# SteveMacenski/slam_toolbox

Measured on NVIDIA B200. Metric: scan matches/sec (1081-beam, +-2m/+-20deg), higher is better.
Workload: dtype u8

## Files before the change

### slam_toolbox_b200/csrc/sm_tile.cu

```cuda
#include <algorithm>
#include <cmath>
#include <cstdlib>
#include <cstring>
#include <type_traits>
#include <vector>

#include "common.cuh"
#include "sm_math.cuh"
#include "sm_types.cuh"
#include "sm_device.cuh"
#include "sm_sweep_dev.cuh"

namespace b200 {

constexpr int kRowTiles = 6;
constexpr int kYTile = 8 * kRowTiles;
constexpr int kChunkBeams = 640;

__device__ __forceinline__ uint32_t smem_u32(const void * p) { return (uint32_t)__cvta_generic_to_shared(p); }
__device__ __forceinline__ void mbar_init(uint32_t bar, uint32_t count)
{
  asm volatile("mbarrier.init.shared::cta.b64 [%0], %1;" ::"r"(bar), "r"(count) : "memory");
}
__device__ __forceinline__ void mbar_expect_tx(uint32_t bar, uint32_t bytes)
{
  asm volatile("mbarrier.arrive.expect_tx.shared::cta.b64 _, [%0], %1;" ::"r"(bar), "r"(bytes) : "memory");
}
__device__ __forceinline__ void bulk_g2s(uint32_t dst, const void * src, uint32_t bytes, uint32_t bar)
{
  asm volatile("cp.async.bulk.shared::cluster.global.mbarrier::complete_tx::bytes [%0], [%1], %2, [%3];" ::"r"(dst), "l"(src),
               "r"(bytes), "r"(bar)
               : "memory");
}
__device__ __forceinline__ void mbar_wait(uint32_t bar, uint32_t parity)
{
  uint32_t done = 0;
  while (!done) {
    asm volatile(
      "{\n\t.reg .pred p;\n\tmbarrier.try_wait.parity.shared::cta.b64 p, [%1], %2;\n\tselp.u32 %0, 1, 0, p;\n\t}"
      : "=r"(done)
      : "r"(bar), "r"(parity)
      : "memory");
  }
}
__device__ __forceinline__ uint32_t cluster_rank()
{
  uint32_t r;
  asm volatile("mov.u32 %0, %%cluster_ctarank;" : "=r"(r));
  return r;
}
__device__ __forceinline__ void cluster_arrive() { asm volatile("barrier.cluster.arrive.release.aligned;" ::: "memory"); }
__device__ __forceinline__ void cluster_wait() { asm volatile("barrier.cluster.wait.acquire.aligned;" ::: "memory"); }
__device__ __forceinline__ uint32_t dsmem_addr(const void * local, uint32_t rank)
{
  uint32_t r;
  asm volatile("mapa.shared::cluster.u32 %0, %1, %2;" : "=r"(r) : "r"(smem_u32(local)), "r"(rank));
  return r;
}
__device__ __forceinline__ void dsmem_st_f64(uint32_t a, double v) { asm volatile("st.shared::cluster.f64 [%0], %1;" ::"r"(a), "d"(v) : "memory"); }
__device__ __forceinline__ void dsmem_st_s32(uint32_t a, int v) { asm volatile("st.shared::cluster.s32 [%0], %1;" ::"r"(a), "r"(v) : "memory"); }
__device__ __forceinline__ int dsmem_ld_s32(uint32_t a)
{
  int v;
  asm volatile("ld.shared::cluster.s32 %0, [%1];" : "=r"(v) : "r"(a) : "memory");
  return v;
}
__device__ __forceinline__ double dsmem_ld_f64(uint32_t a)
{
  double v;
  asm volatile("ld.shared::cluster.f64 %0, [%1];" : "=d"(v) : "r"(a) : "memory");
  return v;
}

__device__ __forceinline__ uint32_t lds_u32(uint32_t a)
{
  uint32_t v;
  asm volatile("ld.shared.u32 %0, [%1];" : "=r"(v) : "r"(a));
  return v;
}

__device__ __forceinline__ uint32_t even_bytes_t(uint32_t w) { return __byte_perm(w, 0, 0x4240); }
__device__ __forceinline__ uint32_t odd_bytes_t(uint32_t w) { return __byte_perm(w, 0, 0x4341); }

struct TieRes {
  double L;
  double L2;
  int cnt;
  int sum0;
  int ties[kMaxTies];
};

__device__ void tie_merge(TieRes & a, const double bL, const double bL2, const int bcnt, const int bsum0, const int * bties)
{
  if (bL == a.L) {
    int out[kMaxTies];
    const int na = a.cnt < kMaxTies ? a.cnt : kMaxTies, nb = bcnt < kMaxTies ? bcnt : kMaxTies;
    int i = 0, j = 0, k = 0;
    while (k < kMaxTies && (i < na || j < nb)) {
      if (j >= nb || (i < na && a.ties[i] < bties[j])) out[k++] = a.ties[i++];
      else out[k++] = bties[j++];
    }
    if (nb > 0 && (na == 0 || bties[0] < a.ties[0])) a.sum0 = bsum0;
    for (int t = 0; t < k; ++t) a.ties[t] = out[t];
    a.cnt += bcnt;
    a.L2 = bL2 > a.L2 ? bL2 : a.L2;
  } else if (bL > a.L) {
    double l2 = a.L > a.L2 ? a.L : a.L2;
    l2 = bL2 > l2 ? bL2 : l2;
    a.L = bL; a.L2 = l2; a.cnt = bcnt; a.sum0 = bsum0;
    const int nb = bcnt < kMaxTies ? bcnt : kMaxTies;
    for (int t = 0; t < nb; ++t) a.ties[t] = bties[t];
// ... 111 lines not shown
        for (int lv = 0; lv < (nlev > 0 ? nlev : 1); ++lv) {
          const uint32_t want = nlev > 0 ? f.level[lv] : 0u;
          for (int it = it0; it < it1; ++it) {
            const int32_t * cl = it == it0 ? cells0 : d.cells + (size_t)it * d.max_n;
            const int ncell = it == it0 ? ncell0 : d.cell_count[it];
            for (int t = tid; t < ncell; t += kTileThreads) {
              const int32_t cell = cl[t];
              if (cell < 0) continue;
              const int cx = (cell & 0xFFFF) + d.roi_x - half, cy = (cell >> 16) + d.roi_y - half;
              for (int ky = (cy ^ pq) & 1; ky < d.ksize; ky += 2) {
                const int rel = ((cy + ky) >> 1) - band_r0;
                if ((unsigned)rel >= (unsigned)f.alloc_rows) continue;
                for (int kx = (cx ^ pp) & 1; kx < d.ksize; kx += 2) {
                  const uint32_t kv = kern[ky * d.ksize + kx];
                  if (nlev > 0) { if (kv == want) S8[rel * pitchB + ((cx + kx) >> 1)] = (uint8_t)kv; }
                  else if (kv) atomic_max_u8(S8 + rel * pitchB + ((cx + kx) >> 1), kv);
                }
              }
            }
          }
          if (lv + 1 < nlev) __syncthreads();
        }
      }
      if (e.flags & (kSeqNewChunk | kSeqNewStage)) __syncthreads();
      if (tid == 0) {
        const TileSeq * nxt = nullptr;
        if (si + 1 < nseq) nxt = seq + si + 1;
        else if (pair + nclusters < d.npairs) nxt = f.seq + f.seq_start[d.pair_query[pair + nclusters] * C + rank];
        if (nxt) issue(nxt, (cnt + 1) & 1);
      }
      mbar_wait(bar0 + 8 * (cnt & 1), (cnt >> 1) & 1);
      const unsigned char * stg = s_raw + f.off_stage + (size_t)(cnt & 1) * f.stage_bytes;
      const int32_t * tbl = reinterpret_cast<const int32_t *>(stg);
      const uint8_t * order = stg + (size_t)e.na * 48;
      const uint16_t * pay = reinterpret_cast<const uint16_t *>(stg + (((size_t)e.na * 52 + 15) & ~(size_t)15));
      const int tiles = f.ytiles * f.xtiles;
      const int nitems = e.na * 4 * tiles;
      const bool has_edge = (e.flags & kSeqHasEdge) != 0;
      for (;;) {
        int item = 0;
        if (lane == 0) item = atomicAdd(&sh.ctr[cnt & 1], 1);
        item = __shfl_sync(0xffffffffu, item, 0);
        if (item >= nitems) break;
        const int gi = item / tiles, ti = item - gi * tiles;
        const int g = order[gi];
        const int al = g >> 2, m = g & 3;
        const int yt = ti / f.xtiles, xt = ti - yt * f.xtiles;
        const int a = e.a0 + al;
        int32_t * Arow = A + (size_t)(a - chunk_a0) * P;
        const int ybase = y_l + kYTile * yt;
       {
        int b = tbl[(al * 4 + m) * 3 + 0];
        const int mb = tbl[(al * 4 + m) * 3 + 1], me = tbl[(al * 4 + m) * 3 + 2];
        const int pe = mb;
        int eb = 0, ee = 0;
        if (has_edge) {
          const int32_t * es = f.edge_start + (((size_t)q * nA + a) * 4 * nb + e.stage) * 4 + m;
          eb = es[0]; ee = es[1];
        }
        if (b == pe && mb == me && eb == ee) break;
        uint32_t base = smem_u32(S8) + (uint32_t)(((y_l + kYTile * yt) * pitch_w + 4 * xt + j_l) * 4);
        asm volatile("" : "+r"(base));
        const int x0 = 4 * (4 * xt + j_l) - m;
        auto flush = [&](const uint32_t (&T0)[kRowTiles], const uint32_t (&T1)[kRowTiles]) {
          uint32_t any = 0;
#pragma unroll
          for (int r = 0; r < kRowTiles; ++r) any |= T0[r] | T1[r];
          if (!__any_sync(0xffffffffu, any != 0)) return;
#pragma unroll
          for (int r = 0; r < kRowTiles; ++r) {
            const int y = ybase + 8 * r;
            if (y >= nY || (T0[r] | T1[r]) == 0) continue;
            int32_t * dst = Arow + y * nX + x0;
            const int v0 = T0[r] & 0xFFFF, v1 = T1[r] & 0xFFFF, v2 = T0[r] >> 16, v3 = T1[r] >> 16;
            if (v0 && (unsigned)(x0 + 0) < (unsigned)nX) atomicAdd(dst + 0, v0);
            if (v1 && (unsigned)(x0 + 1) < (unsigned)nX) atomicAdd(dst + 1, v1);
            if (v2 && (unsigned)(x0 + 2) < (unsigned)nX) atomicAdd(dst + 2, v2);
            if (v3 && (unsigned)(x0 + 3) < (unsigned)nX) atomicAdd(dst + 3, v3);
          }
        };
        bool multi_done = (mb == me);
        if (b < pe || !multi_done) {
          do {
            const int ce = min(pe, b + kChunkBeams);
            uint32_t T0[kRowTiles], T1[kRowTiles];
#pragma unroll
            for (int r = 0; r < kRowTiles; ++r) { T0[r] = 0; T1[r] = 0; }
            for (; b + 3 < ce; b += 4) {
              const uint2 dd = *reinterpret_cast<const uint2 *>(pay + b);
              const uint32_t o0 = base + 4u * __byte_perm(dd.x, 0, 0x4410), o1 = base + 4u * __byte_perm(dd.x, 0, 0x4432);
              const uint32_t o2 = base + 4u * __byte_perm(dd.y, 0, 0x4410), o3 = base + 4u * __byte_perm(dd.y, 0, 0x4432);
#pragma unroll
              for (int r = 0; r < kRowTiles; ++r) {
                const uint32_t wa = lds_u32(o0 + r * 8 * pitchB) +
                                    lds_u32(o1 + r * 8 * pitchB);
                const uint32_t wb = lds_u32(o2 + r * 8 * pitchB) +
                                    lds_u32(o3 + r * 8 * pitchB);
                T0[r] = T0[r] + even_bytes_t(wa) + even_bytes_t(wb);
                T1[r] = T1[r] + odd_bytes_t(wa) + odd_bytes_t(wb);
              }
            }
            for (; b + 1 < ce; b += 2) {
              const uint32_t dd = *reinterpret_cast<const uint32_t *>(pay + b);
              const uint32_t o0 = base + ((dd & 0xFFFFu) << 2), o1 = base + ((dd >> 16) << 2);
#pragma unroll
              for (int r = 0; r < kRowTiles; ++r) {
                const uint32_t w = lds_u32(o0 + r * 8 * pitchB) +
                                   lds_u32(o1 + r * 8 * pitchB);
                T0[r] += even_bytes_t(w);
                T1[r] += odd_bytes_t(w);
              }
            }
            if (b < ce) {
              const uint32_t o0 = base + ((uint32_t)pay[b] << 2);
#pragma unroll
              for (int r = 0; r < kRowTiles; ++r) {
                const uint32_t w = lds_u32(o0 + r * 8 * pitchB);
                T0[r] += even_bytes_t(w);
                T1[r] += odd_bytes_t(w);
              }
              ++b;
            }
            if (b == pe && !multi_done) {
              for (int k = mb; k < me; k += 2) {
                const uint32_t dm = *reinterpret_cast<const uint32_t *>(pay + k);
                const uint32_t o0 = base + ((dm & 0xFFFFu) << 2);
                const uint32_t kk = dm >> 16;
#pragma unroll
                for (int r = 0; r < kRowTiles; ++r) {
                  const uint32_t w = lds_u32(o0 + r * 8 * pitchB);
                  T0[r] += even_bytes_t(w) * kk;
                  T1[r] += odd_bytes_t(w) * kk;
                }
              }
              multi_done = true;
            }
            flush(T0, T1);
          } while (b < pe || !multi_done);
        }
        while (eb < ee) {
          const int ce = min(ee, eb + kChunkBeams);
          uint32_t T0[kRowTiles], T1[kRowTiles];
#pragma unroll
          for (int r = 0; r < kRowTiles; ++r) { T0[r] = 0; T1[r] = 0; }
          for (int b0 = eb; b0 < ce; b0 += 32) {
            const int cn = min(32, ce - b0);
            const int32_t mine = (lane < cn) ? f.edge[b0 + lane] : 0;
            for (int k = 0; k < cn; ++k) {
              const int32_t ev = __shfl_sync(0xffffffffu, mine, k);
              const int row0 = (int)(int16_t)(ev & 0xFFFF) + ybase, wq = (ev >> 16) + 4 * xt + j_l;
              const bool cv = (unsigned)wq < (unsigned)pitch_w;
#pragma unroll
              for (int r = 0; r < kRowTiles; ++r) {
                const int row = row0 + 8 * r;
                const uint32_t w = (cv && (unsigned)row < (unsigned)f.alloc_rows) ? S[row * pitch_w + wq] : 0u;
                T0[r] += even_bytes_t(w);
                T1[r] += odd_bytes_t(w);
              }
            }
          }
          eb = ce;
          flush(T0, T1);
        }
       }
      }
      if (e.flags & kSeqNewStage) {
        const int32_t * ws = f.wrap2_start + ((size_t)q * nA + chunk_a0) * 4 * nb + e.stage;
        const bool has_wrap = (e.flags & kSeqHasWrap) != 0;
        if (has_wrap) {
          for (int p = tid; p < P; p += kTileThreads) {
            const int ex = 2 * (p % nX), ey = 2 * (p / nX);
            for (int al = 0; al < chunk_na; ++al) {
              int acc = 0;
              for (int bi = ws[(size_t)al * 4 * nb]; bi < ws[(size_t)al * 4 * nb + 1]; ++bi) {
                const int32_t ev = f.wrap2[bi];
                const int Xb = (int)(int16_t)(ev & 0xFFFF), Yb = ev >> 16;
                const int col = Xb + ex;
                if ((unsigned)col < (unsigned)d.stride) continue;
                const int r2 = Yb + ey + (col < 0 ? -1 : 1);
                const int c2 = col + (col < 0 ? d.stride : -d.stride);
                if ((unsigned)r2 >= (unsigned)d.height) continue;
                const int rel = (r2 >> 1) - band_r0;
                if ((unsigned)rel >= (unsigned)f.alloc_rows) continue;
                acc += S8[rel * pitchB + (c2 >> 1)];
              }
              if (acc) atomicAdd(A + (size_t)al * P + p, acc);
            }
          }
        }
        const int32_t * ss = f.slow_start + (size_t)q * (nA + 1);
        if (ss[nA] - ss[0] > 0) {
          const int32_t * pos = d.posidx + (size_t)q * P;
          const int own_hi = (band == nb - 1) ? 0x7FFFFFFF : f.band_rows;
          for (int al = 0; al < chunk_na; ++al) {
            const int sb = ss[chunk_a0 + al], se = ss[chunk_a0 + al + 1];
            const int work = (se - sb) * P;
            for (int t = tid; t < work; t += kTileThreads) {
// ... 18 lines not shown
        if (pending_wait) { cluster_wait(); pending_wait = false; }
        double lbest = -1.0;
        int smax = -1;
        if (f.int_ties) {
          for (int p = tid; p < P; p += kTileThreads) {
            int sm = 0;
            for (int al = 0; al < chunk_na; ++al) { const int s = A[(size_t)al * P + p]; sm = s > sm ? s : sm; }
            smax = sm > smax ? sm : smax;
            if (!first_chunk) { const int o = iprobs[p]; sm = o > sm ? o : sm; }
            iprobs[p] = sm;
          }
          for (int o = 16; o > 0; o >>= 1) { const int t = __shfl_xor_sync(0xffffffffu, smax, o); smax = t > smax ? t : smax; }
          __syncthreads();
          if (lane == 0) sh.iscratch[tid >> 5] = smax;
          __syncthreads();
          for (int i = 0; i < kTileThreads / 32; ++i) smax = sh.iscratch[i] > smax ? sh.iscratch[i] : smax;
          __syncthreads();
          lbest = (double)smax;
          lbest /= d.norm;
        } else {
          for (int p = tid; p < P; p += kTileThreads) {
            const int x = p % nX, y = p / nX;
            double pm = first_chunk ? 0.0 : probs[p];
            for (int al = 0; al < chunk_na; ++al) {
              const double r = pose_response(d, q, A[(size_t)al * P + p], x, y, chunk_a0 + al);
              pm = r > pm ? r : pm;
              lbest = r > lbest ? r : lbest;
            }
            probs[p] = pm;
          }
          lbest = block_max(lbest, sh.dscratch);
        }
        const int per = (P + kTileThreads - 1) / kTileThreads;
        const int p0 = min(P, tid * per), p1 = min(P, p0 + per);
        int c = 0;
        for (int p = p0; p < p1; ++p) {
          const int x = p % nX, y = p / nX;
          for (int al = 0; al < chunk_na; ++al) {
            const int s = A[(size_t)al * P + p];
            const bool tie = f.int_ties ? (s == smax) : double_equal(pose_response(d, q, s, x, y, chunk_a0 + al), lbest);
            if (tie) ++c;
          }
        }
        int total = 0;
        int rk = block_exclusive_scan(c, sh.iscratch, total);
        if (c > 0 && rk < kMaxTies) {
          for (int p = p0; p < p1 && rk < kMaxTies; ++p) {
            const int x = p % nX, y = p / nX;
            for (int al = 0; al < chunk_na && rk < kMaxTies; ++al) {
              const int s = A[(size_t)al * P + p];
              const bool tie = f.int_ties ? (s == smax) : double_equal(pose_response(d, q, s, x, y, chunk_a0 + al), lbest);
              if (tie) {
                if (rk == 0) sh.chunk.sum0 = s;
                sh.chunk.ties[rk++] = p * nA + chunk_a0 + al;
              }
            }
          }
        }
        __syncthreads();
        if (tid == 0) {
          if (first_chunk) {
            sh.res.L = lbest; sh.res.L2 = -1e300; sh.res.cnt = total; sh.res.sum0 = sh.chunk.sum0;
            for (int t = 0; t < kMaxTies; ++t) sh.res.ties[t] = sh.chunk.ties[t];
          } else {
            tie_merge(sh.res, lbest, -1e300, total, sh.chunk.sum0, sh.chunk.ties);
          }
        }
// ... 129 lines not shown
    default: return (const void *)k_sweep_tile<0>;
  }
}

static int env_int(const char * name, int dflt)
{
  const char * v = std::getenv(name);
  return (v && *v) ? std::atoi(v) : dflt;
}

static inline bool d_max_n_ok(int max_n) { return max_n > 0 && (max_n & 3) == 0 && max_n <= 4096; }

static inline int floor_div(int a, int b) { return a >= 0 ? a / b : -((-a + b - 1) / b); }

bool build_tile_tables(b200sm * h, SweepHost & S, cudaStream_t st)
{
  const GridGeom & g = h->g;
  const CorrPlan & p0 = S.plans[0];
  const int nX = p0.nX, nY = p0.nY, nA = p0.nA, n = p0.n, nq = S.nq, P = nX * nY;
  TileDev & T = S.tile;
  T = TileDev{};
  for (int i = 0; i < 8; ++i) S.tile_info[i] = 0;
  auto bail = [&](int why) { S.tile_info[5] = why; return false; };
  if (g.order_dependent) return bail(1);
  if ((g.stride & 1) || nA < 1 || nA > 4096) return bail(2);
  for (int q = 0; q < nq; ++q) {
    const CorrPlan & pl = S.plans[q];
    for (int k = 1; k < nX; ++k) if (pl.xs[k] != pl.xs[0] + 2 * k) return bail(6);
    for (int k = 1; k < nY; ++k) if (pl.ys[k] != pl.ys[0] + 2 * k) return bail(7);
  }
  int pitch_w = (g.stride / 2 + 16 + 3) / 4;
  while ((pitch_w & 7) != 4) ++pitch_w;
  const int xtiles = (nX + 3 + 15) / 16, ytiles = (nY + kYTile - 1) / kYTile;
  const int rows_valid = (g.height + 1) / 2;
  const int halo = nY + 2;
  const int base_rows = std::max(1, rows_valid - nY + 1);
  int sms = 148, dev = 0;
  B200_CUDA(cudaGetDevice(&dev));
  B200_CUDA(cudaDeviceGetAttribute(&sms, cudaDevAttrMultiProcessorCount, dev));
  int want_c = h->tile_cluster > 0 ? h->tile_cluster : env_int("B200_SWEEP_CLUSTER", 0);
  if (want_c <= 0) {
    want_c = 1;
    while (want_c < kTileMaxCluster && S.npairs * want_c * 2 <= sms) want_c *= 2;
  }
  int Cc = 1;
  while (Cc * 2 <= std::min(want_c, kTileMaxCluster)) Cc *= 2;
  Cc = std::min(Cc, nA);
  while (Cc & (Cc - 1)) --Cc;
  const int budget = 227 * 1024 - (int)sizeof(TileShared) - 256;
  const int int_ties = (!S.do_penalize && (double)n * kOccupied < 0.9e6) ? 1 : 0;
  const int probs_bytes = (P * (int_ties ? 4 : 8) + 15) & ~15;
  int force_v = h->tile_chunks > 0 ? h->tile_chunks : env_int("B200_SWEEP_CHUNKS", 0);
  int bestV = 0, bestNb = 0, bestB = 0, bestStage = 0;
  long bestCost = -1;
  for (int V = Cc; V <= nA; ++V) {
    if (force_v > 0 && V < std::min(force_v, nA)) continue;
    const int nAc = (nA + V - 1) / V;
    if ((nA + nAc - 1) / nAc != V || nAc > 63) continue;
    const int a_bytes = (nAc * P * 4 + 15) & ~15;
    const int one_angle = 52 + 2 * n + 64;
    int stage = 16 + nAc * 52 + (nAc * n * 2 * 3) / 8 + 64 * nAc;
    stage = std::max(stage, one_angle + 64);
    stage = (stage + 127) & ~127;
    const int s_avail = budget - a_bytes - probs_bytes - 2 * stage;
    if (s_avail <= 0) continue;
    int rows_avail = s_avail / (pitch_w * 4);
    if ((long)rows_avail * pitch_w > 65535) rows_avail = 65535 / pitch_w;
    int B = rows_avail - halo;
    if (B < 8) continue;
    B = std::min(B, base_rows);
    const int nbv = (base_rows + B - 1) / B;
    B = (base_rows + nbv - 1) / nbv;
    const long w_angle = (long)((double)P * n * 0.8 / kTileThreads) + 4L * nbv * (4L * xtiles * ytiles * 100 / 32);
    const long w_raster = 4 * (700 + 3L * std::min(B + halo, rows_valid + halo - nY) * pitch_w / kTileThreads);
    const long cost = (long)((V + Cc - 1) / Cc) * (nbv * w_raster + nAc * w_angle);
    if (bestCost < 0 || cost < bestCost) { bestCost = cost; bestV = V; bestNb = nbv; bestB = B; bestStage = stage; }
  }
  if (bestCost < 0) return bail(4);
  const int V = bestV, nbands = bestNb, B = bestB, nAc = (nA + V - 1) / V, stage_bytes = bestStage;
  const int C = std::min(Cc, V);
  int alloc_rows = std::min(B + halo, rows_valid + halo - nY);
  alloc_rows = std::max(alloc_rows, 1);
  const size_t s_bytes = ((size_t)alloc_rows * pitch_w * 4 + 15) & ~(size_t)15;
  const size_t a_bytes = ((size_t)nAc * P * 4 + 15) & ~(size_t)15;
  T.C = C; T.V = V; T.nAc = nAc; T.nbands = nbands; T.band_rows = B; T.alloc_rows = alloc_rows; T.pitch_w = pitch_w;
  T.xtiles = xtiles; T.ytiles = ytiles; T.stage_bytes = stage_bytes;
  T.int_ties = int_ties;
  {
    std::vector<uint8_t> lv(g.kernel.begin(), g.kernel.end());
    std::sort(lv.begin(), lv.end());
    lv.erase(std::unique(lv.begin(), lv.end()), lv.end());
    if (!lv.empty() && lv[0] == 0) lv.erase(lv.begin());
    T.nlevels = (!lv.empty() && lv.size() <= 4) ? (int)lv.size() : 0;
    for (int i = 0; i < 4; ++i) T.level[i] = i < T.nlevels ? lv[i] : 0;
  }
  T.off_A = s_bytes; T.off_probs = s_bytes + a_bytes; T.off_stage = (T.off_probs + probs_bytes + 127) & ~(size_t)127;
  T.off_cells = T.off_stage + 2 * (size_t)stage_bytes;
  int cell_cap = d_max_n_ok(S.max_n) ? S.max_n : 0;
  if (T.off_cells + 2 * (size_t)cell_cap * 4 + sizeof(TileShared) + 64 > 227 * 1024) cell_cap = 0;
  T.cell_cap = cell_cap;
  size_t smem = T.off_cells + 2 * (size_t)cell_cap * 4;
  const size_t overrun = (size_t)(kYTile * ytiles - nY + 1) * pitch_w * 4;
  if (smem - s_bytes < overrun) smem = s_bytes + overrun;
  if (smem + sizeof(TileShared) + 64 > 227 * 1024) return bail(5);

  const int nstage = 4 * nbands;
  std::vector<uint8_t> blob;
  std::vector<TileSeq> seq;
  std::vector<int32_t> seq_start((size_t)nq * C + 1, 0);
  std::vector<int32_t> edge, edge_start((size_t)nq * nA * nstage * 4 + 1, 0);
  std::vector<int32_t> wrap2, wrap2_start((size_t)nq * nA * nstage + 1, 0);
  std::vector<int32_t> slow, slow_start((size_t)nq * (nA + 1), 0);
  int n_fast = 0, n_edge = 0;
  std::vector<std::vector<uint16_t>> grp((size_t)nA * nstage * 4);
  std::vector<std::vector<int32_t>> egrp((size_t)nA * nstage * 4), wgrp((size_t)nA * nstage);
  blob.reserve((size_t)nq * nA * n * 2 + 4096);
  struct Encoded { int32_t tbl[12]; std::vector<uint16_t> pay; };
  std::vector<Encoded> enc((size_t)nA * nstage);
  std::vector<std::vector<int32_t>> slow_a(nA);
  std::vector<int> nfast_a(nA), nedge_a(nA);
  for (int q = 0; q < nq; ++q) {
    const CorrPlan & pl = S.plans[q];
    const int X0 = pl.xs[0], Y0 = pl.ys[0];
    auto one_angle = [&](int a) {
      for (int k = 0; k < nstage * 4; ++k) { grp[(size_t)a * nstage * 4 + k].clear(); egrp[(size_t)a * nstage * 4 + k].clear(); }
      for (int k = 0; k < nstage; ++k) wgrp[(size_t)a * nstage + k].clear();
      slow_a[a].clear();
      int nf = 0, ne = 0;
      for (int i = 0; i < n; ++i) {
        const int32_t off = pl.offsets[(size_t)a * n + i];
        if (off == kInvalidScan) continue;
        const int gx = pl.ogx[(size_t)a * n + i], gy = pl.ogy[(size_t)a * n + i];
        const int Xb = X0 + gx, Yb = Y0 + gy;
        const bool inside = Xb >= 0 && Xb + 2 * (nX - 1) < g.stride && Yb >= 0 && Yb + 2 * (nY - 1) < g.height;
        if (inside) {
          const int pp = Xb & 1, pq = Yb & 1, c = Xb >> 1, r = Yb >> 1;
          const int band = std::min(r / B, nbands - 1);
          const int wo = (r - band * B) * pitch_w + (c >> 2);
          grp[((size_t)a * nstage + (pq * 2 + pp) * nbands + band) * 4 + (c & 3)].push_back((uint16_t)wo);
          ++nf;
        } else if (Xb >= -g.stride && Xb + 2 * (nX - 1) < 2 * g.stride && Xb > -32768 && Xb < 32767 && Yb > -32768 && Yb < 32767) {
          const bool rows_hit = Yb + 2 * (nY - 1) >= 0 && Yb < g.height;
          const bool cols_hit = Xb + 2 * (nX - 1) >= 0 && Xb < g.stride;
          if (rows_hit && cols_hit) {
            const int c = Xb >> 1, r = Yb >> 1;
            const int band = std::min(std::max(floor_div(r, B), 0), nbands - 1);
            const int rr = r - band * B;
            if (rr > -32768 && rr < 32767) {
              egrp[((size_t)a * nstage + ((Yb & 1) * 2 + (Xb & 1)) * nbands + band) * 4 + (c & 3)].push_back(
                (int32_t)((uint32_t)(rr & 0xFFFF) | ((uint32_t)(c >> 2) << 16)));
              ++ne;
            }
          }
          const bool wraps = Xb < 0 || Xb + 2 * (nX - 1) >= g.stride;
          if (wraps && Yb + 2 * (nY - 1) + 1 >= 0 && Yb - 1 < g.height) {
            const int r = (Yb - 1) >> 1;
            const int band = std::min(std::max(floor_div(r, B), 0), nbands - 1);
            wgrp[(size_t)a * nstage + (((Yb & 1) ^ 1) * 2 + (Xb & 1)) * nbands + band].push_back(
              (int32_t)((uint32_t)(Xb & 0xFFFF) | ((uint32_t)Yb << 16)));
          }
        } else {
          const int32_t dv = device_offset(off, g.data_size);
          if (dv != kDevInvalid) slow_a[a].push_back(dv);
        }
      }
      nfast_a[a] = nf; nedge_a[a] = ne;
      for (int sg = 0; sg < nstage; ++sg) {
        Encoded & E = enc[(size_t)a * nstage + sg];
        std::vector<uint16_t> & pay = E.pay;
        pay.clear();
        for (int m = 0; m < 4; ++m) {
          std::vector<uint16_t> & gk = grp[((size_t)a * nstage + sg) * 4 + m];
          std::sort(gk.begin(), gk.end());
          while (pay.size() & 3) pay.push_back(0);
          const int pb = (int)pay.size();
          const bool dedup = !h->no_dedup && gk.size() <= (size_t)kChunkBeams;
          std::vector<std::pair<uint16_t, uint16_t>> multi;
          for (size_t i = 0; i < gk.size();) {
            size_t j = i;
            while (j < gk.size() && gk[j] == gk[i]) ++j;
            const size_t cnt = j - i;
            if (dedup && cnt >= 3) multi.emplace_back(gk[i], (uint16_t)cnt);
            else for (size_t t = 0; t < cnt; ++t) pay.push_back(gk[i]);
            i = j;
          }
          if (((int)pay.size() - pb) & 1) {
            const uint16_t last = pay.back();
            pay.pop_back();
            multi.emplace_back(last, (uint16_t)1);
          }
          const int mb = (int)pay.size();
          for (auto & mk : multi) { pay.push_back(mk.first); pay.push_back(mk.second); }
          E.tbl[3 * m + 0] = pb; E.tbl[3 * m + 1] = mb; E.tbl[3 * m + 2] = (int)pay.size();
        }
        while (pay.size() & 3) pay.push_back(0);
      }
    };
    host_parallel_for(nA, one_angle);
    for (int a = 0; a < nA; ++a) {
      slow_start[(size_t)q * (nA + 1) + a] = (int32_t)slow.size();
      slow.insert(slow.end(), slow_a[a].begin(), slow_a[a].end());
      n_fast += nfast_a[a]; n_edge += nedge_a[a];
    }
    slow_start[(size_t)q * (nA + 1) + nA] = (int32_t)slow.size();
    for (int a = 0; a < nA; ++a)
      for (int sg = 0; sg < nstage; ++sg) {
        wrap2_start[((size_t)q * nA + a) * nstage + sg] = (int32_t)wrap2.size();
        const auto & w = wgrp[(size_t)a * nstage + sg];
        wrap2.insert(wrap2.end(), w.begin(), w.end());
        for (int m = 0; m < 4; ++m) {
          edge_start[(((size_t)q * nA + a) * nstage + sg) * 4 + m] = (int32_t)edge.size();
          const auto & ev = egrp[((size_t)a * nstage + sg) * 4 + m];
          edge.insert(edge.end(), ev.begin(), ev.end());
        }
      }
    std::vector<uint16_t> pay;
    std::vector<int32_t> tbl;
    for (int r = 0; r < C; ++r) {
      seq_start[(size_t)q * C + r] = (int32_t)seq.size();
      for (int v = r; v < V; v += C) {
        const int ca0 = v * nAc, cna = std::min(nAc, nA - ca0);
        for (int sg = 0; sg < nstage; ++sg) {
          int a = ca0;
          bool first_sub = true;
          do {
            tbl.clear(); pay.clear();
            int na = 0;
            while (a + na < ca0 + cna) {
              const Encoded & E = enc[(size_t)(a + na) * nstage + sg];
              const size_t hdr = (((size_t)(na + 1) * 52) + 15) & ~(size_t)15;
              const size_t bytes = (hdr + (pay.size() + E.pay.size()) * 2 + 15) & ~(size_t)15;
              if (bytes > (size_t)stage_bytes) {
                if (na > 0) break;
                return bail(8);
              }
              const int shift = (int)pay.size();
              for (int k = 0; k < 12; ++k) tbl.push_back(E.tbl[k] + shift);
              pay.insert(pay.end(), E.pay.begin(), E.pay.end());
              ++na;
            }
            const size_t hdr = (((size_t)na * 52) + 15) & ~(size_t)15;
            const size_t bytes = std::max<size_t>(16, (hdr + pay.size() * 2 + 15) & ~(size_t)15);
            TileSeq e{};
            e.off = (int32_t)blob.size();
            e.bytes = (int32_t)bytes;
            e.chunk = (int16_t)v; e.stage = (int16_t)sg; e.a0 = (int16_t)a; e.na = (int16_t)na;
            e.flags = (first_sub ? kSeqNewStage : 0u) | ((first_sub && sg == 0) ? kSeqNewChunk : 0u);
            for (int aa = a; aa < a + na; ++aa)
              for (int m = 0; m < 4; ++m)
                if (!egrp[((size_t)aa * nstage + sg) * 4 + m].empty()) e.flags |= kSeqHasEdge;
            if (first_sub)
              for (int aa = ca0; aa < ca0 + cna; ++aa)
                if (!wgrp[(size_t)aa * nstage + sg].empty()) e.flags |= kSeqHasWrap;
            blob.resize(blob.size() + bytes, 0);
            if (na > 0) {
              std::vector<std::pair<int, int>> wt;
              for (int g2 = 0; g2 < na * 4; ++g2) {
                const int w = (tbl[3 * g2 + 1] - tbl[3 * g2]) + (tbl[3 * g2 + 2] - tbl[3 * g2 + 1]) / 2 +
                              (int)egrp[((size_t)(a + (g2 >> 2)) * nstage + sg) * 4 + (g2 & 3)].size();
                wt.emplace_back(-w, g2);
              }
              std::sort(wt.begin(), wt.end());
              for (int g2 = 0; g2 < na * 4; ++g2) blob[e.off + (size_t)na * 48 + g2] = (uint8_t)wt[g2].second;
              std::memcpy(blob.data() + e.off, tbl.data(), tbl.size() * 4);
              if (!pay.empty()) std::memcpy(blob.data() + e.off + hdr, pay.data(), pay.size() * 2);
            }
            seq.push_back(e);
            a += na;
            first_sub = false;
          } while (a < ca0 + cna);
        }
        seq.back().flags |= kSeqEndChunk;
      }
    }
  }
  seq_start[(size_t)nq * C] = (int32_t)seq.size();
  edge_start[(size_t)nq * nA * nstage * 4] = (int32_t)edge.size();
  wrap2_start[(size_t)nq * nA * nstage] = (int32_t)wrap2.size();
  edge.push_back(0); wrap2.push_back(0); slow.push_back(0);
  blob.resize(blob.size() + 16, 0);

  auto up = [&](auto & dst, const auto & src) {
    using TT = typename std::remove_reference<decltype(src)>::type::value_type;
    dst.reserve(src.size());
    sweep_stage_h2d(dst.p, src.data(), src.size() * sizeof(TT), st);
  };
  up(S.d_tile_desc, blob);
  up(S.d_tile_seq, seq);
  up(S.d_tile_seq_start, seq_start);
  up(S.d_tile_edge, edge);
  up(S.d_tile_edge_start, edge_start);
  up(S.d_tile_wrap2, wrap2);
  up(S.d_tile_wrap2_start, wrap2_start);
  up(S.d_tile_slow, slow);
  up(S.d_tile_slow_start, slow_start);
  T.desc = S.d_tile_desc.p; T.seq = S.d_tile_seq.p; T.seq_start = S.d_tile_seq_start.p;
  T.edge = S.d_tile_edge.p; T.edge_start = S.d_tile_edge_start.p;
  T.wrap2 = S.d_tile_wrap2.p; T.wrap2_start = S.d_tile_wrap2_start.p;
  T.slow = S.d_tile_slow.p; T.slow_start = S.d_tile_slow_start.p;
  T.enabled = 1;
  S.tile_smem = smem;
// ... 45 lines not shown
```

### slam_toolbox_b200/csrc/sm_types.cuh

```cuda
#pragma once
#include <cstdint>
#include <functional>
#include <utility>
#include <vector>

#include "common.cuh"
#include "sm_math.cuh"

namespace b200 {

constexpr int kMaxTies = 24;
constexpr int kSweepThreads = 512;
constexpr int32_t kDevInvalid = -(1 << 30);

struct GridGeom {
  int width = 0, height = 0, stride = 0;
  int roi_x = 0, roi_y = 0, roi_w = 0, roi_h = 0;
  int data_size = 0;
  int ksize = 0;
  bool order_dependent = false;
  double scale = 0.0;
  double off_x = 0.0, off_y = 0.0;
  std::vector<uint8_t> kernel;
};
// ... 79 lines not shown
constexpr int kSubPitchW = 76;
constexpr int kFastRowTiles = 6;
constexpr int kFastChunk = 640;
struct FastDev {
  int enabled;
  int sub_rows;
  int xtiles;
  const uint16_t * beams;
  const uint16_t * mult;
  const int32_t * cls_start;
  const int32_t * edge;
  const int32_t * edge_start;
  const int32_t * wrap2;
  const int32_t * wrap2_start;
  const int32_t * slow;
  const int32_t * slow_start;
};

constexpr int kTileThreads = 1024;
constexpr int kTileMaxCluster = 8;
struct TileSeq {
  int32_t off;
  int32_t bytes;
  int16_t chunk, stage;
  int16_t a0, na;
  uint32_t flags;
};
constexpr uint32_t kSeqNewChunk = 1, kSeqNewStage = 2, kSeqEndChunk = 4, kSeqHasEdge = 8, kSeqHasWrap = 16;
struct TileDev {
  int enabled;
  int C, V, nAc;
  int nbands, band_rows, alloc_rows, pitch_w;
  int xtiles, ytiles;
  int stage_bytes;
  int nlevels;
  uint32_t level[4];
  int int_ties;
  size_t off_A, off_probs, off_stage, off_cells;
  int cell_cap;
  const uint8_t * desc;
  const TileSeq * seq;
  const int32_t * seq_start;
  const int32_t * edge;
  const int32_t * edge_start;
  const int32_t * wrap2;
  const int32_t * wrap2_start;
  const int32_t * slow;
  const int32_t * slow_start;
};

struct FineDev {
  int P, nA;
  const int32_t * offsets;
  const int32_t * posidx;
  int32_t * sums;
};

struct SweepHost {
  bool uploaded = false, ran = false;
  int nq = 0, npairs = 0, nitems = 0, nscans = 0, max_n = 0, n = 0, blocks = 0;
  bool do_penalize = false;
  std::vector<CorrPlan> plans;
  std::vector<int32_t> pair_query, pair_chain;
  std::vector<b200_scan> queries, scans;
  std::vector<int32_t> chain_start;
  DevBuf<int32_t> d_offsets, d_posidx, d_scan_pt_start, d_pair_query, d_pair_chain, d_pair_item_start, d_item_pair, d_item_scan,
// ... 82 lines not shown
```

Before: 430,700.

## Compute fast-path correlation sums with u8 tensor-core MMA instead of byte-lane adds

Replaces the per-tile scalar byte-lane accumulation of the in-bounds beam path with mma.sync m16n8k32 u8 instructions. Beam offsets are re-encoded on the host as 16-row quad steps with a deduplicated multiplicity weight packed into B-fragment bytes, so repeated cells are folded into the MMA. Work items become per-angle y-group by x-range tiles. Host staging and stage sizing are redone for the new 64-byte step layout, and angles can be split across stage segments. This trades the simpler scalar path for more complex encoding and padded steps, in order to raise arithmetic throughput.

```diff
diff --git a/slam_toolbox_b200/csrc/sm_tile.cu b/slam_toolbox_b200/csrc/sm_tile.cu
--- a/slam_toolbox_b200/csrc/sm_tile.cu
+++ b/slam_toolbox_b200/csrc/sm_tile.cu
@@ -16,6 +16,7 @@
 constexpr int kRowTiles = 6;
 constexpr int kYTile = 8 * kRowTiles;
 constexpr int kChunkBeams = 640;
+constexpr int kTileSlots = 6;
 
 __device__ __forceinline__ uint32_t smem_u32(const void * p) { return (uint32_t)__cvta_generic_to_shared(p); }
 __device__ __forceinline__ void mbar_init(uint32_t bar, uint32_t count)
@@ -77,6 +78,13 @@
   uint32_t v;
   asm volatile("ld.shared.u32 %0, [%1];" : "=r"(v) : "r"(a));
   return v;
+}
+
+__device__ __forceinline__ void mma_u8(int (&c)[4], uint32_t a0, uint32_t a1, uint32_t a2, uint32_t a3, uint32_t b0, uint32_t b1)
+{
+  asm("mma.sync.aligned.m16n8k32.row.col.s32.u8.u8.s32 {%0, %1, %2, %3}, {%4, %5, %6, %7}, {%8, %9}, {%0, %1, %2, %3};"
+      : "+r"(c[0]), "+r"(c[1]), "+r"(c[2]), "+r"(c[3])
+      : "r"(a0), "r"(a1), "r"(a2), "r"(a3), "r"(b0), "r"(b1));
 }
 
 __device__ __forceinline__ uint32_t even_bytes_t(uint32_t w) { return __byte_perm(w, 0, 0x4240); }
@@ -254,112 +262,72 @@
       mbar_wait(bar0 + 8 * (cnt & 1), (cnt >> 1) & 1);
       const unsigned char * stg = s_raw + f.off_stage + (size_t)(cnt & 1) * f.stage_bytes;
       const int32_t * tbl = reinterpret_cast<const int32_t *>(stg);
-      const uint8_t * order = stg + (size_t)e.na * 48;
-      const uint16_t * pay = reinterpret_cast<const uint16_t *>(stg + (((size_t)e.na * 52 + 15) & ~(size_t)15));
+      const uint8_t * order = stg + (size_t)e.na * 12;
+      const uint4 * steps = reinterpret_cast<const uint4 *>(stg + (((size_t)e.na * 13 + 15) & ~(size_t)15));
+      const int per_angle = f.ygroups * f.wranges;
+      const int fast_items = e.na * per_angle;
       const int tiles = f.ytiles * f.xtiles;
-      const int nitems = e.na * 4 * tiles;
-      const bool has_edge = (e.flags & kSeqHasEdge) != 0;
+      const int nitems = fast_items + ((e.flags & kSeqHasEdge) ? e.na * 4 * tiles : 0);
       for (;;) {
         int item = 0;
         if (lane == 0) item = atomicAdd(&sh.ctr[cnt & 1], 1);
         item = __shfl_sync(0xffffffffu, item, 0);
         if (item >= nitems) break;
-        const int gi = item / tiles, ti = item - gi * tiles;
-        const int g = order[gi];
-        const int al = g >> 2, m = g & 3;
+        if (item < fast_items) {
+          const int gi = item / per_angle, ti = item - gi * per_angle;
+          const int al = order[gi];
+          const int s0 = tbl[3 * al], s1 = tbl[3 * al + 1];
+          if (s0 == s1) continue;
+          const int yg = ti / f.wranges, wr = ti - yg * f.wranges;
+          const int g = lane >> 2, t4 = lane & 3;
+          uint32_t base = smem_u32(S8) + (uint32_t)(((16 * yg + g) * pitch_w + kTileSlots * wr) * 4);
+          asm volatile("" : "+r"(base));
+          uint32_t sel = 0;
+#pragma unroll
+          for (int j = 0; j < 4; ++j) {
+            const int k = j + 4 - g;
+            sel |= (uint32_t)((k >= 0 && k <= 3) ? k : 4) << (4 * j);
+          }
+          int acc[kTileSlots][4];
+#pragma unroll
+          for (int s = 0; s < kTileSlots; ++s) acc[s][0] = acc[s][1] = acc[s][2] = acc[s][3] = 0;
+          const uint4 * de = steps + 4 * s1;
+          for (const uint4 * dp = steps + 4 * s0 + t4; dp < de; dp += 4) {
+            const uint4 dd = *dp;
+            const uint32_t oa = base + dd.x, ob = base + dd.y;
+            const uint32_t b0 = __byte_perm(dd.z, 0, sel), b1 = __byte_perm(dd.w, 0, sel);
+#pragma unroll
+            for (int s = 0; s < kTileSlots; ++s)
+              mma_u8(acc[s], lds_u32(oa + 4 * s), lds_u32(oa + 4 * s + 8 * pitchB), lds_u32(ob + 4 * s), lds_u32(ob + 4 * s + 8 * pitchB),
+                     b0, b1);
+          }
+          int32_t * Arow = A + (size_t)(e.a0 + al - chunk_a0) * P;
+#pragma unroll
+          for (int s = 0; s < kTileSlots; ++s) {
+            const int x = 4 * (kTileSlots * wr + s) - 4 + 2 * t4;
+#pragma unroll
+            for (int hh = 0; hh < 2; ++hh) {
+              const int y = 16 * yg + g + 8 * hh;
+              if (y >= nY) continue;
+              if (acc[s][2 * hh] && (unsigned)x < (unsigned)nX) atomicAdd(Arow + y * nX + x, acc[s][2 * hh]);
+              if (acc[s][2 * hh + 1] && (unsigned)(x + 1) < (unsigned)nX) atomicAdd(Arow + y * nX + x + 1, acc[s][2 * hh + 1]);
+            }
+          }
+          continue;
+        }
+        const int ei = item - fast_items;
+        const int gi = ei / tiles, ti = ei - gi * tiles;
+        const int al = gi >> 2, m = gi & 3;
+        if (!tbl[3 * al + 2]) continue;
+        const int a = e.a0 + al;
+        const int32_t * es = f.edge_start + (((size_t)q * nA + a) * 4 * nb + e.stage) * 4 + m;
+        int eb = es[0];
+        const int ee = es[1];
+        if (eb == ee) continue;
         const int yt = ti / f.xtiles, xt = ti - yt * f.xtiles;
-        const int a = e.a0 + al;
         int32_t * Arow = A + (size_t)(a - chunk_a0) * P;
         const int ybase = y_l + kYTile * yt;
-       {
-        int b = tbl[(al * 4 + m) * 3 + 0];
-        const int mb = tbl[(al * 4 + m) * 3 + 1], me = tbl[(al * 4 + m) * 3 + 2];
-        const int pe = mb;
-        int eb = 0, ee = 0;
-        if (has_edge) {
-          const int32_t * es = f.edge_start + (((size_t)q * nA + a) * 4 * nb + e.stage) * 4 + m;
-          eb = es[0]; ee = es[1];
-        }
-        if (b == pe && mb == me && eb == ee) break;
-        uint32_t base = smem_u32(S8) + (uint32_t)(((y_l + kYTile * yt) * pitch_w + 4 * xt + j_l) * 4);
-        asm volatile("" : "+r"(base));
         const int x0 = 4 * (4 * xt + j_l) - m;
-        auto flush = [&](const uint32_t (&T0)[kRowTiles], const uint32_t (&T1)[kRowTiles]) {
-          uint32_t any = 0;
-#pragma unroll
-          for (int r = 0; r < kRowTiles; ++r) any |= T0[r] | T1[r];
-          if (!__any_sync(0xffffffffu, any != 0)) return;
-#pragma unroll
-          for (int r = 0; r < kRowTiles; ++r) {
-            const int y = ybase + 8 * r;
-            if (y >= nY || (T0[r] | T1[r]) == 0) continue;
-            int32_t * dst = Arow + y * nX + x0;
-            const int v0 = T0[r] & 0xFFFF, v1 = T1[r] & 0xFFFF, v2 = T0[r] >> 16, v3 = T1[r] >> 16;
-            if (v0 && (unsigned)(x0 + 0) < (unsigned)nX) atomicAdd(dst + 0, v0);
-            if (v1 && (unsigned)(x0 + 1) < (unsigned)nX) atomicAdd(dst + 1, v1);
-            if (v2 && (unsigned)(x0 + 2) < (unsigned)nX) atomicAdd(dst + 2, v2);
-            if (v3 && (unsigned)(x0 + 3) < (unsigned)nX) atomicAdd(dst + 3, v3);
-          }
-        };
-        bool multi_done = (mb == me);
-        if (b < pe || !multi_done) {
-          do {
-            const int ce = min(pe, b + kChunkBeams);
-            uint32_t T0[kRowTiles], T1[kRowTiles];
-#pragma unroll
-            for (int r = 0; r < kRowTiles; ++r) { T0[r] = 0; T1[r] = 0; }
-            for (; b + 3 < ce; b += 4) {
-              const uint2 dd = *reinterpret_cast<const uint2 *>(pay + b);
-              const uint32_t o0 = base + 4u * __byte_perm(dd.x, 0, 0x4410), o1 = base + 4u * __byte_perm(dd.x, 0, 0x4432);
-              const uint32_t o2 = base + 4u * __byte_perm(dd.y, 0, 0x4410), o3 = base + 4u * __byte_perm(dd.y, 0, 0x4432);
-#pragma unroll
-              for (int r = 0; r < kRowTiles; ++r) {
-                const uint32_t wa = lds_u32(o0 + r * 8 * pitchB) +
-                                    lds_u32(o1 + r * 8 * pitchB);
-                const uint32_t wb = lds_u32(o2 + r * 8 * pitchB) +
-                                    lds_u32(o3 + r * 8 * pitchB);
-                T0[r] = T0[r] + even_bytes_t(wa) + even_bytes_t(wb);
-                T1[r] = T1[r] + odd_bytes_t(wa) + odd_bytes_t(wb);
-              }
-            }
-            for (; b + 1 < ce; b += 2) {
-              const uint32_t dd = *reinterpret_cast<const uint32_t *>(pay + b);
-              const uint32_t o0 = base + ((dd & 0xFFFFu) << 2), o1 = base + ((dd >> 16) << 2);
-#pragma unroll
-              for (int r = 0; r < kRowTiles; ++r) {
-                const uint32_t w = lds_u32(o0 + r * 8 * pitchB) +
-                                   lds_u32(o1 + r * 8 * pitchB);
-                T0[r] += even_bytes_t(w);
-                T1[r] += odd_bytes_t(w);
-              }
-            }
-            if (b < ce) {
-              const uint32_t o0 = base + ((uint32_t)pay[b] << 2);
-#pragma unroll
-              for (int r = 0; r < kRowTiles; ++r) {
-                const uint32_t w = lds_u32(o0 + r * 8 * pitchB);
-                T0[r] += even_bytes_t(w);
-                T1[r] += odd_bytes_t(w);
-              }
-              ++b;
-            }
-            if (b == pe && !multi_done) {
-              for (int k = mb; k < me; k += 2) {
-                const uint32_t dm = *reinterpret_cast<const uint32_t *>(pay + k);
-                const uint32_t o0 = base + ((dm & 0xFFFFu) << 2);
-                const uint32_t kk = dm >> 16;
-#pragma unroll
-                for (int r = 0; r < kRowTiles; ++r) {
-                  const uint32_t w = lds_u32(o0 + r * 8 * pitchB);
-                  T0[r] += even_bytes_t(w) * kk;
-                  T1[r] += odd_bytes_t(w) * kk;
-                }
-              }
-              multi_done = true;
-            }
-            flush(T0, T1);
-          } while (b < pe || !multi_done);
-        }
         while (eb < ee) {
           const int ce = min(ee, eb + kChunkBeams);
           uint32_t T0[kRowTiles], T1[kRowTiles];
@@ -382,9 +350,22 @@
             }
           }
           eb = ce;
-          flush(T0, T1);
-        }
-       }
+          uint32_t any = 0;
+#pragma unroll
+          for (int r = 0; r < kRowTiles; ++r) any |= T0[r] | T1[r];
+          if (!__any_sync(0xffffffffu, any != 0)) continue;
+#pragma unroll
+          for (int r = 0; r < kRowTiles; ++r) {
+            const int y = ybase + 8 * r;
+            if (y >= nY || (T0[r] | T1[r]) == 0) continue;
+            int32_t * dst = Arow + y * nX + x0;
+            const int v0 = T0[r] & 0xFFFF, v1 = T1[r] & 0xFFFF, v2 = T0[r] >> 16, v3 = T1[r] >> 16;
+            if (v0 && (unsigned)(x0 + 0) < (unsigned)nX) atomicAdd(dst + 0, v0);
+            if (v1 && (unsigned)(x0 + 1) < (unsigned)nX) atomicAdd(dst + 1, v1);
+            if (v2 && (unsigned)(x0 + 2) < (unsigned)nX) atomicAdd(dst + 2, v2);
+            if (v3 && (unsigned)(x0 + 3) < (unsigned)nX) atomicAdd(dst + 3, v3);
+          }
+        }
       }
       if (e.flags & kSeqNewStage) {
         const int32_t * ws = f.wrap2_start + ((size_t)q * nA + chunk_a0) * 4 * nb + e.stage;
@@ -469,7 +450,9 @@
           lbest = block_max(lbest, sh.dscratch);
         }
         const int per = (P + kTileThreads - 1) / kTileThreads;
-        const int p0 = min(P, tid * per), p1 = min(P, p0 + per);
+        int t_own;
+        asm volatile("mov.u32 %0, %%tid.x;" : "=r"(t_own));
+        const int p0 = min(P, t_own * per), p1 = min(P, p0 + per);
         int c = 0;
         for (int p = p0; p < p1; ++p) {
           const int x = p % nX, y = p / nX;
@@ -665,6 +648,7 @@
   int pitch_w = (g.stride / 2 + 16 + 3) / 4;
   while ((pitch_w & 7) != 4) ++pitch_w;
   const int xtiles = (nX + 3 + 15) / 16, ytiles = (nY + kYTile - 1) / kYTile;
+  const int ygroups = (nY + 15) / 16, wranges = ((nX + 2) / 4 + 1 + kTileSlots - 1) / kTileSlots;
   const int rows_valid = (g.height + 1) / 2;
   const int halo = nY + 2;
   const int base_rows = std::max(1, rows_valid - nY + 1);
@@ -691,20 +675,21 @@
     const int nAc = (nA + V - 1) / V;
     if ((nA + nAc - 1) / nAc != V || nAc > 63) continue;
     const int a_bytes = (nAc * P * 4 + 15) & ~15;
-    const int one_angle = 52 + 2 * n + 64;
-    int stage = 16 + nAc * 52 + (nAc * n * 2 * 3) / 8 + 64 * nAc;
-    stage = std::max(stage, one_angle + 64);
-    stage = (stage + 127) & ~127;
-    const int s_avail = budget - a_bytes - probs_bytes - 2 * stage;
-    if (s_avail <= 0) continue;
-    int rows_avail = s_avail / (pitch_w * 4);
-    if ((long)rows_avail * pitch_w > 65535) rows_avail = 65535 / pitch_w;
-    int B = rows_avail - halo;
-    if (B < 8) continue;
-    B = std::min(B, base_rows);
-    const int nbv = (base_rows + B - 1) / B;
-    B = (base_rows + nbv - 1) / nbv;
-    const long w_angle = (long)((double)P * n * 0.8 / kTileThreads) + 4L * nbv * (4L * xtiles * ytiles * 100 / 32);
+    int stage = 0, B = 0, nbv = 1;
+    bool fits = true;
+    for (int pass = 0; pass < 2 && fits; ++pass) {
+      stage = 16 + nAc * 13 + (nAc * n * 3) / (2 * nbv) + 64 * nAc;
+      stage = std::max(stage, 16 + 13 + 64 * 16);
+      stage = (stage + 127) & ~127;
+      const int s_avail = budget - a_bytes - probs_bytes - 2 * stage;
+      B = s_avail / (pitch_w * 4) - halo;
+      if (s_avail <= 0 || B < 8) { fits = false; break; }
+      B = std::min(B, base_rows);
+      nbv = (base_rows + B - 1) / B;
+      B = (base_rows + nbv - 1) / nbv;
+    }
+    if (!fits) continue;
+    const long w_angle = (long)((double)P * n * 0.4 / kTileThreads) + 4L * nbv * ((long)ygroups * wranges * 100 / 32);
     const long w_raster = 4 * (700 + 3L * std::min(B + halo, rows_valid + halo - nY) * pitch_w / kTileThreads);
     const long cost = (long)((V + Cc - 1) / Cc) * (nbv * w_raster + nAc * w_angle);
     if (bestCost < 0 || cost < bestCost) { bestCost = cost; bestV = V; bestNb = nbv; bestB = B; bestStage = stage; }
@@ -717,7 +702,7 @@
   const size_t s_bytes = ((size_t)alloc_rows * pitch_w * 4 + 15) & ~(size_t)15;
   const size_t a_bytes = ((size_t)nAc * P * 4 + 15) & ~(size_t)15;
   T.C = C; T.V = V; T.nAc = nAc; T.nbands = nbands; T.band_rows = B; T.alloc_rows = alloc_rows; T.pitch_w = pitch_w;
-  T.xtiles = xtiles; T.ytiles = ytiles; T.stage_bytes = stage_bytes;
+  T.xtiles = xtiles; T.ytiles = ytiles; T.ygroups = ygroups; T.wranges = wranges; T.stage_bytes = stage_bytes;
   T.int_ties = int_ties;
   {
     std::vector<uint8_t> lv(g.kernel.begin(), g.kernel.end());
@@ -733,7 +718,8 @@
   if (T.off_cells + 2 * (size_t)cell_cap * 4 + sizeof(TileShared) + 64 > 227 * 1024) cell_cap = 0;
   T.cell_cap = cell_cap;
   size_t smem = T.off_cells + 2 * (size_t)cell_cap * 4;
-  const size_t overrun = (size_t)(kYTile * ytiles - nY + 1) * pitch_w * 4;
+  const size_t overrun = std::max((size_t)(kYTile * ytiles - nY + 1) * pitch_w * 4,
+                                  ((size_t)(16 * ygroups - nY + 1) * pitch_w + (size_t)kTileSlots * wranges) * 4);
   if (smem - s_bytes < overrun) smem = s_bytes + overrun;
   if (smem + sizeof(TileShared) + 64 > 227 * 1024) return bail(5);
 
@@ -745,10 +731,10 @@
   std::vector<int32_t> wrap2, wrap2_start((size_t)nq * nA * nstage + 1, 0);
   std::vector<int32_t> slow, slow_start((size_t)nq * (nA + 1), 0);
   int n_fast = 0, n_edge = 0;
-  std::vector<std::vector<uint16_t>> grp((size_t)nA * nstage * 4);
+  std::vector<std::vector<uint32_t>> grp((size_t)nA * nstage);
   std::vector<std::vector<int32_t>> egrp((size_t)nA * nstage * 4), wgrp((size_t)nA * nstage);
   blob.reserve((size_t)nq * nA * n * 2 + 4096);
-  struct Encoded { int32_t tbl[12]; std::vector<uint16_t> pay; };
+  struct Encoded { int steps; std::vector<uint32_t> pay; };
   std::vector<Encoded> enc((size_t)nA * nstage);
   std::vector<std::vector<int32_t>> slow_a(nA);
   std::vector<int> nfast_a(nA), nedge_a(nA);
@@ -756,8 +742,8 @@
     const CorrPlan & pl = S.plans[q];
     const int X0 = pl.xs[0], Y0 = pl.ys[0];
     auto one_angle = [&](int a) {
-      for (int k = 0; k < nstage * 4; ++k) { grp[(size_t)a * nstage * 4 + k].clear(); egrp[(size_t)a * nstage * 4 + k].clear(); }
-      for (int k = 0; k < nstage; ++k) wgrp[(size_t)a * nstage + k].clear();
+      for (int k = 0; k < nstage * 4; ++k) egrp[(size_t)a * nstage * 4 + k].clear();
+      for (int k = 0; k < nstage; ++k) { grp[(size_t)a * nstage + k].clear(); wgrp[(size_t)a * nstage + k].clear(); }
       slow_a[a].clear();
       int nf = 0, ne = 0;
       for (int i = 0; i < n; ++i) {
@@ -770,7 +756,7 @@
           const int pp = Xb & 1, pq = Yb & 1, c = Xb >> 1, r = Yb >> 1;
           const int band = std::min(r / B, nbands - 1);
           const int wo = (r - band * B) * pitch_w + (c >> 2);
-          grp[((size_t)a * nstage + (pq * 2 + pp) * nbands + band) * 4 + (c & 3)].push_back((uint16_t)wo);
+          grp[(size_t)a * nstage + (pq * 2 + pp) * nbands + band].push_back(((uint32_t)wo << 2) | (uint32_t)(c & 3));
           ++nf;
         } else if (Xb >= -g.stride && Xb + 2 * (nX - 1) < 2 * g.stride && Xb > -32768 && Xb < 32767 && Yb > -32768 && Yb < 32767) {
           const bool rows_hit = Yb + 2 * (nY - 1) >= 0 && Yb < g.height;
@@ -799,34 +785,34 @@
       }
       nfast_a[a] = nf; nedge_a[a] = ne;
       for (int sg = 0; sg < nstage; ++sg) {
+        std::vector<uint32_t> & gk = grp[(size_t)a * nstage + sg];
+        std::sort(gk.begin(), gk.end());
+        std::vector<uint32_t> bk[4][2];
+        for (size_t i = 0; i < gk.size();) {
+          size_t j = i;
+          while (j < gk.size() && gk[j] == gk[i]) ++j;
+          const uint32_t wo = gk[i] >> 2, m = gk[i] & 3;
+          for (size_t t = i; t < j;) {
+            const uint32_t w = h->no_dedup ? 1u : (uint32_t)std::min<size_t>(j - t, 255);
+            bk[wo & 3][0].push_back(4u * wo);
+            bk[wo & 3][1].push_back(w << (8 * m));
+            t += w;
+          }
+          i = j;
+        }
+        size_t quads = 0;
+        for (int r = 0; r < 4; ++r) quads = std::max(quads, bk[r][0].size());
+        quads = (quads + 1) & ~(size_t)1;
         Encoded & E = enc[(size_t)a * nstage + sg];
-        std::vector<uint16_t> & pay = E.pay;
-        pay.clear();
-        for (int m = 0; m < 4; ++m) {
-          std::vector<uint16_t> & gk = grp[((size_t)a * nstage + sg) * 4 + m];
-          std::sort(gk.begin(), gk.end());
-          while (pay.size() & 3) pay.push_back(0);
-          const int pb = (int)pay.size();
-          const bool dedup = !h->no_dedup && gk.size() <= (size_t)kChunkBeams;
-          std::vector<std::pair<uint16_t, uint16_t>> multi;
-          for (size_t i = 0; i < gk.size();) {
-            size_t j = i;
-            while (j < gk.size() && gk[j] == gk[i]) ++j;
-            const size_t cnt = j - i;
-            if (dedup && cnt >= 3) multi.emplace_back(gk[i], (uint16_t)cnt);
-            else for (size_t t = 0; t < cnt; ++t) pay.push_back(gk[i]);
-            i = j;
-          }
-          if (((int)pay.size() - pb) & 1) {
-            const uint16_t last = pay.back();
-            pay.pop_back();
-            multi.emplace_back(last, (uint16_t)1);
-          }
-          const int mb = (int)pay.size();
-          for (auto & mk : multi) { pay.push_back(mk.first); pay.push_back(mk.second); }
-          E.tbl[3 * m + 0] = pb; E.tbl[3 * m + 1] = mb; E.tbl[3 * m + 2] = (int)pay.size();
-        }
-        while (pay.size() & 3) pay.push_back(0);
+        E.steps = (int)(quads / 2);
+        E.pay.assign(quads * 8, 0u);
+        for (size_t qd = 0; qd < quads; ++qd)
+          for (int r = 0; r < 4; ++r) {
+            const bool real = qd < bk[r][0].size();
+            uint32_t * d = E.pay.data() + (qd / 2) * 16 + r * 4 + (qd & 1);
+            d[0] = real ? bk[r][0][qd] : 4u * (uint32_t)r;
+            d[2] = real ? bk[r][1][qd] : 0u;
+          }
       }
     };
     host_parallel_for(nA, one_angle);
@@ -847,59 +833,61 @@
           edge.insert(edge.end(), ev.begin(), ev.end());
         }
       }
-    std::vector<uint16_t> pay;
-    std::vector<int32_t> tbl;
+    struct Seg { int a, k0, k1; };
+    std::vector<Seg> segs;
     for (int r = 0; r < C; ++r) {
       seq_start[(size_t)q * C + r] = (int32_t)seq.size();
       for (int v = r; v < V; v += C) {
         const int ca0 = v * nAc, cna = std::min(nAc, nA - ca0);
         for (int sg = 0; sg < nstage; ++sg) {
-          int a = ca0;
+          int a = ca0, k = 0;
           bool first_sub = true;
           do {
-            tbl.clear(); pay.clear();
-            int na = 0;
-            while (a + na < ca0 + cna) {
-              const Encoded & E = enc[(size_t)(a + na) * nstage + sg];
-              const size_t hdr = (((size_t)(na + 1) * 52) + 15) & ~(size_t)15;
-              const size_t bytes = (hdr + (pay.size() + E.pay.size()) * 2 + 15) & ~(size_t)15;
-              if (bytes > (size_t)stage_bytes) {
-                if (na > 0) break;
-                return bail(8);
-              }
-              const int shift = (int)pay.size();
-              for (int k = 0; k < 12; ++k) tbl.push_back(E.tbl[k] + shift);
-              pay.insert(pay.end(), E.pay.begin(), E.pay.end());
-              ++na;
-            }
-            const size_t hdr = (((size_t)na * 52) + 15) & ~(size_t)15;
-            const size_t bytes = std::max<size_t>(16, (hdr + pay.size() * 2 + 15) & ~(size_t)15);
+            segs.clear();
+            long used = 0;
+            while (a < ca0 + cna) {
+              const Encoded & E = enc[(size_t)a * nstage + sg];
+              const long room = ((long)stage_bytes - (long)((((segs.size() + 1) * 13) + 15) & ~(size_t)15)) / 64 - used;
+              if (room < 0 || (room == 0 && E.steps > k)) break;
+              const int take = (int)std::min<long>(E.steps - k, room);
+              segs.push_back({a, k, k + take});
+              used += take;
+              k += take;
+              if (k < E.steps) break;
+              ++a; k = 0;
+            }
+            if (segs.empty()) return bail(8);
+            const int na = (int)segs.size();
+            const size_t hdr = (((size_t)na * 13) + 15) & ~(size_t)15;
+            const size_t bytes = hdr + (size_t)used * 64;
             TileSeq e{};
             e.off = (int32_t)blob.size();
             e.bytes = (int32_t)bytes;
-            e.chunk = (int16_t)v; e.stage = (int16_t)sg; e.a0 = (int16_t)a; e.na = (int16_t)na;
+            e.chunk = (int16_t)v; e.stage = (int16_t)sg; e.a0 = (int16_t)segs[0].a; e.na = (int16_t)na;
             e.flags = (first_sub ? kSeqNewStage : 0u) | ((first_sub && sg == 0) ? kSeqNewChunk : 0u);
-            for (int aa = a; aa < a + na; ++aa)
+            for (const Seg & sgm : segs)
               for (int m = 0; m < 4; ++m)
-                if (!egrp[((size_t)aa * nstage + sg) * 4 + m].empty()) e.flags |= kSeqHasEdge;
+                if (sgm.k0 == 0 && !egrp[((size_t)sgm.a * nstage + sg) * 4 + m].empty()) e.flags |= kSeqHasEdge;
             if (first_sub)
               for (int aa = ca0; aa < ca0 + cna; ++aa)
                 if (!wgrp[(size_t)aa * nstage + sg].empty()) e.flags |= kSeqHasWrap;
             blob.resize(blob.size() + bytes, 0);
-            if (na > 0) {
-              std::vector<std::pair<int, int>> wt;
-              for (int g2 = 0; g2 < na * 4; ++g2) {
-                const int w = (tbl[3 * g2 + 1] - tbl[3 * g2]) + (tbl[3 * g2 + 2] - tbl[3 * g2 + 1]) / 2 +
-                              (int)egrp[((size_t)(a + (g2 >> 2)) * nstage + sg) * 4 + (g2 & 3)].size();
-                wt.emplace_back(-w, g2);
-              }
-              std::sort(wt.begin(), wt.end());
-              for (int g2 = 0; g2 < na * 4; ++g2) blob[e.off + (size_t)na * 48 + g2] = (uint8_t)wt[g2].second;
-              std::memcpy(blob.data() + e.off, tbl.data(), tbl.size() * 4);
-              if (!pay.empty()) std::memcpy(blob.data() + e.off + hdr, pay.data(), pay.size() * 2);
-            }
+            int32_t * tbl = reinterpret_cast<int32_t *>(blob.data() + e.off);
+            uint8_t * order = blob.data() + e.off + (size_t)na * 12;
+            uint32_t * steps = reinterpret_cast<uint32_t *>(blob.data() + e.off + hdr);
+            std::vector<std::pair<int, int>> wt;
+            int at = 0;
+            for (int i = 0; i < na; ++i) {
+              const Seg & sgm = segs[i];
+              const int len = sgm.k1 - sgm.k0;
+              tbl[3 * i + 0] = at; tbl[3 * i + 1] = at + len; tbl[3 * i + 2] = sgm.k0 == 0;
+              if (len) std::memcpy(steps + (size_t)at * 16, enc[(size_t)sgm.a * nstage + sg].pay.data() + (size_t)sgm.k0 * 16, (size_t)len * 64);
+              at += len;
+              wt.emplace_back(-len, i);
+            }
+            std::sort(wt.begin(), wt.end());
+            for (int i = 0; i < na; ++i) order[i] = (uint8_t)wt[i].second;
             seq.push_back(e);
-            a += na;
             first_sub = false;
           } while (a < ca0 + cna);
         }
diff --git a/slam_toolbox_b200/csrc/sm_types.cuh b/slam_toolbox_b200/csrc/sm_types.cuh
--- a/slam_toolbox_b200/csrc/sm_types.cuh
+++ b/slam_toolbox_b200/csrc/sm_types.cuh
@@ -135,6 +135,7 @@
   int C, V, nAc;
   int nbands, band_rows, alloc_rows, pitch_w;
   int xtiles, ytiles;
+  int ygroups, wranges;
   int stage_bytes;
   int nlevels;
   uint32_t level[4];
```

New measurement: 521,700 (median of 6 runs). 1.21x the previous value.
